# ZKI-PH-ImageAnalysis/seq2squiggle

Measured on AMD Instinct MI355X. Metric: signal samples/sec at 5 kb reads (padded [chunks x 250] samples the predict path emits), higher is better.
Workload: dtype f16x3

## Files before the change

include/s2s_hip.h:

```cpp
#ifndef S2S_HIP_H
#define S2S_HIP_H

#include <stddef.h>
#include <stdint.h>

#ifdef __cplusplus
extern "C" {
#endif

#define S2S_OK 0
#define S2S_ERR_ARG (-1)
#define S2S_ERR_HIP (-2)
#define S2S_ERR_BLOB (-3)
#define S2S_ERR_CODEC (-4)

#define S2S_MODE_F32 0
#define S2S_MODE_F16X3 1
#define S2S_MODE_F16 3
#define S2S_MODE_GENERIC 4
#define S2S_MODE_GENERIC_F16 5
#define S2S_MODE_GENERIC_GEOMETRY 6
#define S2S_MODE_GENERIC_GEOMETRY_F16 7
#define S2S_GEOMETRY_MAX_DNA_LEN 64
#define S2S_GEOMETRY_MAX_SIGNAL_LEN 1024
// ... 252 lines not shown

int64_t s2s_sampler_replay_law(uint32_t* mt_state, const int64_t* contig_ends, int32_t n_contigs,
                               const int64_t* const* n_pos, const int64_t* n_pos_count, int64_t num_seqs, int64_t first_read_i, int64_t r,
                               uint64_t seed, int64_t total_len, int32_t is_dna, int32_t min_read_len, int32_t max_retries,
                               int64_t stop_after, int32_t law, int32_t* out_lengths, int64_t* out_next_read_i);
int64_t s2s_length_law(int32_t law, uint32_t seed, double r, int64_t total_len);

int64_t s2s_fasta_count(const uint8_t* data, int64_t n);
int64_t s2s_fastq_clean(const uint8_t* data, int64_t n, int32_t map_acgtn, uint8_t* out, int64_t* seq_offs,
                        int64_t* name_span, int64_t max_records);
int64_t s2s_fasta_clean(const uint8_t* data, int64_t n, int32_t map_acgtn, uint8_t* out, int64_t* seq_offs,
                        int64_t* name_span, int64_t max_records);

int64_t s2s_copy_ranges(int32_t n, const int32_t* src_fd, const int64_t* src_off, const int32_t* dst_fd, const int64_t* dst_off,
                        const int64_t* len, int32_t threads, int32_t engine);
int64_t s2s_blow5_scan(int32_t fd, int64_t begin, int64_t end);
int64_t s2s_blow5_scan_upto(int32_t fd, int64_t begin, int64_t limit, int64_t max_records, int64_t* out_end);

#define S2S_ATTENTION_REDO_THRESHOLD 0.055
double s2s_attention_redo_threshold(void);
int s2s_set_attention_path(s2s_handle* h, int32_t path);
int s2s_get_attention_path(const s2s_handle* h, int32_t* path, double* calibration_redo_rate);

int s2s_stats_read(s2s_handle* h, uint64_t* out10);

int s2s_diag_read(s2s_handle* h, uint64_t* out384);

#define S2S_TRAINER_DEFAULT_MEMORY ((size_t)2 << 30)
typedef struct s2s_trainer s2s_trainer;
typedef struct s2s_adam {
    double lr, beta1, beta2, eps, weight_decay;
    double clip;
    int32_t decoupled;
    int32_t step;
} s2s_adam;
int s2s_trainer_create(const s2s_config* cfg, const void* weights_blob, size_t blob_bytes, int device, s2s_trainer** out);
void s2s_trainer_destroy(s2s_trainer* t);
const char* s2s_trainer_last_error(const s2s_trainer* t);
int s2s_trainer_set_memory(s2s_trainer* t, size_t bytes);
int64_t s2s_trainer_micro_batch(const s2s_trainer* t, int32_t B);
int s2s_trainer_weights(s2s_trainer* t, void* stream, float* out_blob);
int s2s_trainer_gradients(s2s_trainer* t, void* stream, const uint8_t* kmers, const int32_t* dwell, const float* target,
                          const float* stdev, int32_t B, float* out_loss, float* out_grad);
int s2s_trainer_step(s2s_trainer* t, void* stream, const uint8_t* kmers, const int32_t* dwell, const float* target,
                     const float* stdev, int32_t B, const s2s_adam* hyper, float* out_stats);

// ... 5 lines not shown
```

seq2squiggle_amd/_lib.py:

```python
import ctypes as C
import os

from ._build import LIB as _LIB_DEFAULT

_lib = None
loaded_before_torch = False


class S2SConfig(C.Structure):
    _fields_ = [("seq_kmer", C.c_int32), ("max_dna_len", C.c_int32), ("max_signal_len", C.c_int32),
                ("dmodel", C.c_int32), ("dff", C.c_int32), ("n_heads", C.c_int32), ("encoder_layers", C.c_int32),
                ("decoder_layers", C.c_int32), ("pre_layers", C.c_int32), ("scaling_max_value", C.c_float),
                ("compute_mode", C.c_int32), ("decoder_heads", C.c_int32)]


class S2SParams(C.Structure):
    _fields_ = [("dwell_mean", C.c_float), ("dwell_std", C.c_float), ("noise_std", C.c_float),
                ("min_noise", C.c_float), ("min_duration", C.c_float), ("noise_sampling", C.c_int32),
                ("duration_sampling", C.c_int32), ("seed", C.c_uint64)]


class S2SDebug(C.Structure):
    _fields_ = [(n, C.c_void_p) for n in ("emb_out", "enc_out", "sigma", "conc", "rate", "g", "y_scaled", "z01", "emb_in", "dec_in")]


class S2SAdam(C.Structure):
    _fields_ = [("lr", C.c_double), ("beta1", C.c_double), ("beta2", C.c_double), ("eps", C.c_double), ("weight_decay", C.c_double),
                ("clip", C.c_double), ("decoupled", C.c_int32), ("step", C.c_int32)]


EXPORTS = ("s2s_blob_floats", "s2s_create", "s2s_destroy", "s2s_last_error", "s2s_predict_chunks", "s2s_predict_packed",
           "s2s_export_reads", "s2s_svb_encode", "s2s_philox_u32", "s2s_set_profiling", "s2s_get_kernel_ms", "s2s_stats_read", "s2s_set_attention_path", "s2s_get_attention_path", "s2s_diag_read",
           "s2s_blow5_pack_bound", "s2s_blow5_pack", "s2s_compress_rows", "s2s_sampler_replay", "s2s_sampler_replay_law", "s2s_length_law",
           "s2s_fasta_count", "s2s_fasta_clean", "s2s_fastq_clean", "s2s_copy_ranges", "s2s_blow5_scan", "s2s_blow5_scan_upto", "s2s_attention_redo_threshold", "s2s_evaluate_chunks",
           "s2s_align_chunks", "s2s_paf_format", "s2s_paf_format_bound", "s2s_event_stats", "s2s_events_format", "s2s_events_format_bound",
           "s2s_kmer_table_rows", "s2s_kmer_table_accumulate", "s2s_kmer_table_format", "s2s_kmer_table_format_bound",
           "s2s_event_fixed", "s2s_kmer_model_accumulate", "s2s_kmer_model_format", "s2s_kmer_model_format_bound",
           "s2s_dtw_max_band", "s2s_signal_median_mad", "s2s_signal_normalise", "s2s_dtw_banded",
           "s2s_signal_median_mad_host", "s2s_signal_normalise_host", "s2s_dtw_banded_host",
           "s2s_dtw_path_scratch_bytes", "s2s_dtw_path", "s2s_dtw_path_host",
           "s2s_sdtw_max_query", "s2s_sdtw", "s2s_sdtw_host",
           "s2s_resquiggle_scratch_bytes", "s2s_resquiggle", "s2s_event_sums", "s2s_resquiggle_host", "s2s_event_sums_host",
           "s2s_segment_capacity", "s2s_segment_scratch_bytes", "s2s_segment", "s2s_segment_host", "s2s_segment_format_bound",
           "s2s_segment_format",
           "s2s_eventalign_scratch_bytes", "s2s_event_means", "s2s_eventalign", "s2s_event_means_host", "s2s_eventalign_host",
           "s2s_chunk_scratch_bytes", "s2s_chunk_pack", "s2s_chunk_pack_host",
           "s2s_kmer_model_events", "s2s_kmer_model_events_host",
           "s2s_trainer_create", "s2s_trainer_destroy", "s2s_trainer_last_error", "s2s_trainer_set_memory", "s2s_trainer_micro_batch",
           "s2s_trainer_weights", "s2s_trainer_gradients", "s2s_trainer_step")


def lib():
    global _lib
    if _lib is not None:
        return _lib
# ... 13 lines not shown
            fn = getattr(L, name)
        except AttributeError:
            if lenient:
                return
            raise
        fn.restype, fn.argtypes = restype, argtypes
    bind("s2s_blob_floats", C.c_size_t, [C.POINTER(S2SConfig)])
    bind("s2s_create", i32, [C.POINTER(S2SConfig), vp, C.c_size_t, i32, C.POINTER(vp)])
    bind("s2s_destroy", None, [vp])
    bind("s2s_last_error", C.c_char_p, [vp])
    bind("s2s_predict_chunks", i32, [vp, vp, vp, vp, i64, i32, C.POINTER(S2SParams), vp, vp, vp, vp, vp,
                                     C.POINTER(S2SDebug)])
    bind("s2s_evaluate_chunks", i32, [vp, vp, vp, vp, vp, vp, i32, vp, vp, C.POINTER(S2SDebug)])
    bind("s2s_predict_packed", i32, [vp, vp, vp, vp, vp, i64, i32, C.POINTER(S2SParams), vp, vp])
    bind("s2s_export_reads", i32, [vp, vp, vp, i32, vp, i32, vp, vp, vp, i64, f32, f32, f32, i32])
    bind("s2s_svb_encode", i32, [vp, vp, vp, vp, vp, vp, i32, i64, i32, vp, i64, vp])
    bind("s2s_philox_u32", i32, [vp, vp, u64, u32, u32, u32, u32, i32, vp])
    bind("s2s_set_profiling", i32, [vp, i32])
    bind("s2s_get_kernel_ms", i32, [vp, C.POINTER(C.c_double), C.POINTER(i64), C.POINTER(i64)])
    bind("s2s_stats_read", i32, [vp, C.POINTER(C.c_uint64)])
    bind("s2s_set_attention_path", i32, [vp, i32])
    bind("s2s_get_attention_path", i32, [vp, C.POINTER(i32), C.POINTER(C.c_double)])
    bind("s2s_diag_read", i32, [vp, C.POINTER(C.c_uint64)])
    bind("s2s_blow5_pack_bound", i64, [i64, i32])
    bind("s2s_blow5_pack", i64, [vp, vp, vp, vp, vp, vp, i32, i32, i32, i32, vp, i64])
    bind("s2s_compress_rows", i64, [vp, vp, i32, i32, i32, i32, vp, i64, vp])
    bind("s2s_sampler_replay", i64, [vp, vp, i32, vp, vp, i64, i64, i64, u64, i64, i32, i32, i32, i64, vp, vp])
    bind("s2s_sampler_replay_law", i64, [vp, vp, i32, vp, vp, i64, i64, i64, u64, i64, i32, i32, i32, i64, i32, vp, vp])
    bind("s2s_length_law", i64, [i32, u32, C.c_double, i64])
    bind("s2s_fastq_clean", i64, [vp, i64, i32, vp, vp, vp, i64])
    bind("s2s_fasta_count", i64, [vp, i64])
    bind("s2s_fasta_clean", i64, [vp, i64, i32, vp, vp, vp, i64])
    bind("s2s_copy_ranges", i64, [i32, vp, vp, vp, vp, vp, i32, i32])
    bind("s2s_blow5_scan", i64, [i32, i64, i64])
    bind("s2s_blow5_scan_upto", i64, [i32, i64, i64, i64, C.POINTER(i64)])
    bind("s2s_attention_redo_threshold", C.c_double, [])
    bind("s2s_align_chunks", i32, [vp, vp, vp, vp, i32, vp])
    bind("s2s_paf_format_bound", i64, [i64, i32, i32, i64])
    bind("s2s_paf_format", i64, [vp, i32, vp, vp, vp, i32, vp, vp, i32, i32, i32, vp, i64])
    bind("s2s_event_stats", i32, [vp, vp, vp, vp, i32, f32, f32, f32, vp, vp, vp])
    bind("s2s_events_format_bound", i64, [i64, i32, i64, i32, f32, f32, f32, i64, i32])
    bind("s2s_events_format", i64, [vp, vp, vp, i32, vp, vp, vp, i32, vp, vp, i32, vp, vp, i32, f32, f32, f32, vp, i32, i32, i32, vp, i64])
    bind("s2s_kmer_table_rows", i64, [i32])
    bind("s2s_kmer_table_accumulate", i32, [vp, vp, vp, vp, vp, vp, vp, i32, f32, f32, f32, vp])
    bind("s2s_kmer_table_format_bound", i64, [vp, i32, f32, f32, f32, i32])
    bind("s2s_kmer_table_format", i64, [vp, i32, f32, f32, f32, i32, vp, i64])
# ... 50 lines not shown
```

seq2squiggle_amd/csrc/s2s_device.h:

```cpp
#pragma once
#include <hip/hip_runtime.h>
#include <stdint.h>

typedef float f32x4 __attribute__((ext_vector_type(4)));
typedef float f32x2 __attribute__((ext_vector_type(2)));

#define S2S_MAX_LAYERS 4

struct LayerOff {
    int stream;
    int stream_h;
    int stream_f;
    int bq, bk, bv, bfc, b1, b2;
    int bq_nat, bk_nat;
    int ln1g, ln1b, ln2g, ln2b;
};
struct MlpOff { int w0, b0, w3, b3, w0h; };
struct ModelDev {
    int k, enc_layers, dec_layers, pre_layers;
    float scale;
    int pe_enc, pe_dec;
    int emb_wt, emb_b;
    int pre_w[S2S_MAX_LAYERS], pre_b[S2S_MAX_LAYERS], pre_wh[S2S_MAX_LAYERS];
    LayerOff enc[S2S_MAX_LAYERS], dec[S2S_MAX_LAYERS];
// ... 24 lines not shown
#define DIAG_STAMP(slot)                                                            \
    do {                                                                            \
        __builtin_amdgcn_sched_barrier(0);                                          \
        const unsigned long long n_ = __builtin_readcyclecounter();                 \
        if ((threadIdx.x & 63) == 0) s2s_diag_lds[(threadIdx.x >> 6) * S2S_DIAG_SLOTS + (slot)] += n_ - diag_t_; \
        diag_t_ = n_;                                                               \
        __builtin_amdgcn_sched_barrier(0);                                          \
    } while (0)
#define DIAG_COUNT(slot, n) do { if ((threadIdx.x & 63) == 0) s2s_diag_lds[(threadIdx.x >> 6) * S2S_DIAG_SLOTS + (slot)] += (n); } while (0)
#elif defined(S2S_STAMP_SB)
#define DIAG_DECL
#define DIAG_STAMP(slot) __builtin_amdgcn_sched_barrier(0)
#define DIAG_COUNT(slot, n)
#else
#define DIAG_DECL
#define DIAG_STAMP(slot)
#define DIAG_COUNT(slot, n)
#endif

#define S2S_STAT_REDO 0
#define S2S_STAT_CYCLES 1
#define S2S_STAT_TICKS 2
#define S2S_STAT_WGS 3
__shared__ __attribute__((aligned(256))) unsigned s2s_stats_lds[64];

#ifdef S2S_TILEHIST
__shared__ unsigned s2s_hist_lds[2 * 2 * 64];
#endif
constexpr int S2S_STATIC_LDS_BYTES = 256
#ifdef S2S_DIAG
    + 8 * S2S_DIAG_SLOTS * 8
#endif
#ifdef S2S_TILEHIST
    + 2 * 2 * 64 * 4
#endif
    ;

#ifndef S2S_ABL
#define S2S_ABL 0
#endif
#define MFMA4(a, b, c) __builtin_amdgcn_mfma_f32_16x16x4f32((a), (b), (c), 0, 0, 0)

__device__ __forceinline__ f32x4 ldg4(const float* p) { return *reinterpret_cast<const f32x4*>(p); }
__device__ __forceinline__ void store_stream(float* p, float v) { __hip_atomic_store(p, v, __ATOMIC_RELAXED, __HIP_MEMORY_SCOPE_AGENT); }
__device__ __forceinline__ void store_stream(int* p, int v) { __hip_atomic_store(p, v, __ATOMIC_RELAXED, __HIP_MEMORY_SCOPE_AGENT); }
__device__ __forceinline__ float sum_g(float v) {
    const unsigned u = __float_as_uint(v);
// ... 364 lines not shown
```

seq2squiggle_amd/csrc/s2s_hip.hip:

```cpp
#include "s2s_device.h"
#include "s2s_device_h.h"
#include "s2s_generic.h"
#include "s2s_generic_h.h"
#include "s2s_train.h"
#include "../../include/s2s_hip.h"
#include "s2s_event_fixed.h"
#define S2S_DTW_KERNELS
#include "s2s_dtw.h"
#include "s2s_sdtw.h"
#include "s2s_resquiggle.h"
#include "s2s_prims.h"
#include "s2s_segment.h"
#include "s2s_eventalign.h"
#include "s2s_chunk.h"
#include "s2s_kmer_model_events.h"

#include <cctype>
#include <cstdio>
#include <cstdlib>
#include <cstring>
#include <immintrin.h>
#include <map>
#include <mutex>
#include <string>
// ... 392 lines not shown
                                 ? __fmul_rn(__fmul_rn(fmaxf(se, P.min_noise), P.noise_std), M.scale)
                                 : P.noise_std;
            if (y != 0.0f) y = mul_then_add(z, sd, y);
        }
        store_stream(out_signal + t, fmaxf(y, 0.0f));
    }
}

template <int MODE> struct Fused {
    static constexpr int FMODE = (MODE == 3) ? 1 : MODE;
    static constexpr int FNQ = (FMODE == 1) ? 2 : 1;
    static constexpr int GROUP = DEC_WAVES * FNQ;
    static constexpr bool PF = (MODE == 1);
    static constexpr int LDS = (MODE == 0) ? DEC_LDS_F32 : DEC_LDS_H + (S2S_SLOT_FLOATS + S2S_SV_FLOATS + S2S_PROG_INTS + S2S_Z2_FLOATS) * 4;
    static_assert(LDS + S2S_STATIC_LDS_BYTES + 16 <= 160 * 1024, "LDS per workgroup: dynamic + the static arrays in front of it");
    static_assert(FMODE == 1 || DEC_WAVES * FrontLdsF32::BYTES <= LDS, "the f32 frontend waves' K/V images share the decoder's LDS");
};
#define S2S_MAX_GROUP (2 * DEC_WAVES)
template <int MODE, bool TEST, bool EXACT = false>
__global__ __launch_bounds__(DEC_WAVES * 64, DEC_WPS) void s2s_fused_kernel(
    const ModelDev M, const float* __restrict__ W, const uint8_t* __restrict__ bases,
    const long long* __restrict__ chunk_start, const uint8_t* __restrict__ n_valid, int n_chunks, long long first_chunk,
    ParamsDev P, const float* __restrict__ inj_g_, const float* __restrict__ inj_zdw_, const float* __restrict__ inj_z01_,
    float* __restrict__ handoff, int* __restrict__ out_dur, float* __restrict__ out_signal, DebugDev dbg_, long long dbg_base) {
    using F = Fused<MODE>;
    const float* const inj_g = TEST ? inj_g_ : nullptr;
    const float* const inj_zdw = TEST ? inj_zdw_ : nullptr;
    const float* const inj_z01 = TEST ? inj_z01_ : nullptr;
    DebugDev dbg = dbg_;
    if (!TEST) { dbg = DebugDev{}; dbg.diag = dbg_.diag; dbg.stats = dbg_.stats; }
    extern __shared__ __attribute__((aligned(16))) char lds_raw[];
    const int wave = __builtin_amdgcn_readfirstlane(threadIdx.x >> 6);
    const int lane = threadIdx.x & 63;
    const int nb = S2S_T_ENC + M.k - 1;
    if constexpr (MODE != 0) att32_consts<AttnLdsH<DEC_NQ, DEC_WAVES, DEC_NKT>>(lds_raw, threadIdx.x, DEC_WAVES * 64);
    if constexpr (MODE != 0) {
        if (threadIdx.x < S2S_PROG_INTS + S2S_Z2_FLOATS)
            reinterpret_cast<int*>(lds_raw + DEC_LDS_H + (S2S_SLOT_FLOATS + S2S_SV_FLOATS) * 4)[threadIdx.x] = 0;
    }
    if (threadIdx.x == 0) {
        const unsigned long long c0 = __builtin_readcyclecounter(), r0 = __builtin_amdgcn_s_memrealtime();
        s2s_stats_lds[0] = 0;
        s2s_stats_lds[4] = (unsigned)c0; s2s_stats_lds[5] = (unsigned)(c0 >> 32);
        s2s_stats_lds[6] = (unsigned)r0; s2s_stats_lds[7] = (unsigned)(r0 >> 32);
    }
#ifdef S2S_TILEHIST
    for (int i = threadIdx.x; i < 2 * 2 * 64; i += DEC_WAVES * 64) s2s_hist_lds[i] = 0;
#endif
#ifdef S2S_DIAG
    for (int i = threadIdx.x; i < 8 * S2S_DIAG_SLOTS; i += DEC_WAVES * 64) s2s_diag_lds[i] = 0;
    const unsigned long long diag_c0 = __builtin_readcyclecounter(), diag_r0 = __builtin_amdgcn_s_memrealtime();
    __syncthreads();
#endif
    float* const slot0 = handoff + (size_t)blockIdx.x * S2S_MAX_GROUP * S2S_SLOT_FLOATS;
    const int lo = (int)((long long)blockIdx.x * n_chunks / gridDim.x), hi = (int)((long long)(blockIdx.x + 1) * n_chunks / gridDim.x);
#pragma unroll 1
    for (int g0 = lo; g0 < hi; g0 += F::GROUP) {
        const int n_here = hi - g0 < F::GROUP ? hi - g0 : F::GROUP;
        float one = 1.0f;
        asm volatile("" : "+s"(one));
        DIAG_DECL;
        __syncthreads();
        {
            int lnf = lane;
            asm volatile("" : "+v"(lnf));
            auto chunk_of = [&](const int j, const int j_filler) {
                const bool live = j < n_here;
                const int b = g0 + (live ? j : j_filler);
                return FrontChunk{chunk_start ? bases + chunk_start[b] : bases + (size_t)b * nb, n_valid[b],
                                  (unsigned long long)(first_chunk + b), inj_g ? inj_g + (size_t)b * 16 : nullptr,
                                  inj_zdw ? inj_zdw + (size_t)b * 16 : nullptr, slot0 + j * S2S_SLOT_FLOATS,
                                  out_dur + (size_t)b * 16, dbg_base + b, live};
            };
            if constexpr (F::FMODE == 1) {
                if (n_here > DEC_WAVES) {
                    const FrontChunk io[2] = {chunk_of(2 * wave, 2 * wave), chunk_of(2 * wave + 1, 2 * wave)};
                    if (2 * wave < n_here) frontend_h16<2>(M, W, io, P, dbg, lnf, one);
                } else {
                    const FrontChunk io[1] = {chunk_of(wave, 0)};
                    if (wave < n_here) frontend_h16<1>(M, W, io, P, dbg, lnf, one);
                }
            } else {
                const FrontChunk io[1] = {chunk_of(wave, 0)};
                if (wave < n_here) frontend_f32(M, W, io, P, lds_raw + wave * FrontLdsF32::BYTES, dbg, lnf);
            }
        }
        __syncthreads();
        DIAG_STAMP(7);
        f32x4 X[DEC_NQ][4];
        float sig_ext[DEC_NQ];
        {
            int lg = lane;
            asm volatile("" : "+v"(lg));
            GatherRaw R;
            dec_gather_issue(M, W, slot0, wave, lg, R);
            dec_gather_finish(R, wave, lg, X, sig_ext);
            if (TEST && dbg.dec_in) dec_override(dbg.dec_in, dbg_base + g0, wave, lg, X);
        }
        DIAG_STAMP(8);
#pragma unroll 1
        for (int j = 0; j < ((S2S_ABL & 65536) ? 0 : n_here); ++j) {
            const int b = g0 + j;
            const float* next = slot0 + (j + 1 < n_here ? j + 1 : j) * S2S_SLOT_FLOATS;
            dec_blocks<MODE, EXACT>(M, W, X, lds_raw, wave, lane, one, dbg.diag, F::PF ? next : nullptr);
            DIAG_STAMP(15);
            int ln = lane;
            asm volatile("" : "+v"(ln));
            float ys, se;
            dec_project(M, W, X, sig_ext, ln, ys, se);
            GatherRaw R;
            if constexpr (F::PF) dec_gather_issue(M, W, reinterpret_cast<const float*>(lds_raw + DEC_LDS_H), wave, ln, R);
// ... 5 lines not shown
            DIAG_STAMP(9);
        }
    }
#ifdef S2S_DIAG
    DIAG_COUNT(16, __builtin_readcyclecounter() - diag_c0);
    DIAG_COUNT(17, __builtin_amdgcn_s_memrealtime() - diag_r0);
    DIAG_COUNT(18, 1ull);
    __syncthreads();
    if (dbg.diag)
        for (int i = threadIdx.x; i < 8 * S2S_DIAG_SLOTS; i += DEC_WAVES * 64)
            if (s2s_diag_lds[i]) atomicAdd(dbg.diag + i, s2s_diag_lds[i]);
#endif
    __syncthreads();
#ifdef S2S_TILEHIST
    if (dbg.diag)
        for (int i = threadIdx.x; i < 2 * 2 * 64; i += DEC_WAVES * 64)
            if (s2s_hist_lds[i]) atomicAdd(dbg.diag + i, (unsigned long long)s2s_hist_lds[i]);
#endif
    if (threadIdx.x == 0 && dbg.stats) {
        const unsigned long long c0 = ((unsigned long long)s2s_stats_lds[5] << 32) | s2s_stats_lds[4];
        const unsigned long long r0 = ((unsigned long long)s2s_stats_lds[7] << 32) | s2s_stats_lds[6];
        if (s2s_stats_lds[0]) atomicAdd(dbg.stats + S2S_STAT_REDO, (unsigned long long)s2s_stats_lds[0]);
        atomicAdd(dbg.stats + S2S_STAT_CYCLES, __builtin_readcyclecounter() - c0);
        atomicAdd(dbg.stats + S2S_STAT_TICKS, __builtin_amdgcn_s_memrealtime() - r0);
        atomicAdd(dbg.stats + S2S_STAT_WGS, 1ull);
    }
}

template <int MODE, bool EXACT>
__global__ __launch_bounds__(DEC_WAVES * 64, DEC_WPS) void s2s_eval_kernel(
    const ModelDev M, const float* __restrict__ W, const uint8_t* __restrict__ kmers, const int* __restrict__ dwell, int n_chunks,
    ParamsDev P, float* __restrict__ handoff, float* __restrict__ y, DebugDev dbg_) {
    using F = Fused<MODE>;
    extern __shared__ __attribute__((aligned(16))) char lds_raw[];
    const int wave = __builtin_amdgcn_readfirstlane(threadIdx.x >> 6);
    const int lane = threadIdx.x & 63;
    if constexpr (MODE != 0) att32_consts<AttnLdsH<DEC_NQ, DEC_WAVES, DEC_NKT>>(lds_raw, threadIdx.x, DEC_WAVES * 64);
    if constexpr (MODE != 0) {
        if (threadIdx.x < S2S_PROG_INTS + S2S_Z2_FLOATS)
            reinterpret_cast<int*>(lds_raw + DEC_LDS_H + (S2S_SLOT_FLOATS + S2S_SV_FLOATS) * 4)[threadIdx.x] = 0;
    }
    if (threadIdx.x == 0) s2s_stats_lds[0] = 0;
    DebugDev dbg{};
    dbg.sigma = dbg_.sigma; dbg.conc = dbg_.conc; dbg.rate = dbg_.rate;
    float* const slot0 = handoff + (size_t)blockIdx.x * S2S_MAX_GROUP * S2S_SLOT_FLOATS;
    const int lo = (int)((long long)blockIdx.x * n_chunks / gridDim.x), hi = (int)((long long)(blockIdx.x + 1) * n_chunks / gridDim.x);
    const int kb = S2S_T_ENC * M.k;
#pragma unroll 1
// ... 569 lines not shown

struct s2s_handle {
    s2s_config cfg;
    int device = 0;
    ModelDev model;
    char* slab = nullptr;
    size_t slab_bytes = 0;
    float* d_arena = nullptr;
    size_t arena_floats = 0;
    int tile = 0;
    int n_wg = 256;
    float* handoff = nullptr;
    int* ws_counts = nullptr;
    long long* ws_offs = nullptr;
    int ws_export_cap = 0;
    int* ws_svb = nullptr;
    int ws_svb_cap = 0;
    bool profiling = false;
    unsigned long long* d_diag = nullptr;
    unsigned long long* d_stats = nullptr;
    long long stat_chunks = 0;
    int attn_exact = 0;
    long long stat_exact_chunks = 0;
    double calib_redo_rate = -1.0;
    std::vector<EventPair> events;
    std::string err;
    struct Generic {
        int d = 0, dff = 0, h_enc = 0, h_dec = 0;
        int te = 16, ts = 250;
        bool f16 = false;
        long long pe_enc = 0, pe_dec = 0, emb_wt = 0, emb_b = 0, out_w = 0, out_b = 0, w0cat = 0, b0cat = 0;
        long long pre_w[S2S_MAX_LAYERS] = {}, pre_b[S2S_MAX_LAYERS] = {};
        GenLayer enc[S2S_MAX_LAYERS] = {}, dec[S2S_MAX_LAYERS] = {};
        GenLayerH dech[S2S_MAX_LAYERS] = {};
        GenHeads heads = {};
        int ld_d = 0, ld_f = 0;
        int slice_max = 0;
        float* ws = nullptr;
        int ws_chunks = 0;
    } gen;
    float* ev_ws = nullptr;
    int ev_chunks = 0;
};

namespace {

// ... 515 lines not shown
    if ((e = hipMemcpy(h->d_arena, A.v.data(), h->arena_floats * sizeof(float), hipMemcpyHostToDevice)) != hipSuccess)
        return bail(e, "hipMemcpy(arena)");
    if ((e = hipMemset(h->d_stats, 0, 256)) != hipSuccess) return bail(e, "hipMemset(stats)");
    const struct { const void* fn; int bytes; } dyn_lds[] = {
        {reinterpret_cast<const void*>(s2s_fused_kernel<0, false>), Fused<0>::LDS}, {reinterpret_cast<const void*>(s2s_fused_kernel<1, false>), Fused<1>::LDS},
        {reinterpret_cast<const void*>(s2s_fused_kernel<3, false>), Fused<3>::LDS}, {reinterpret_cast<const void*>(s2s_fused_kernel<0, true>), Fused<0>::LDS},
        {reinterpret_cast<const void*>(s2s_fused_kernel<1, true>), Fused<1>::LDS},  {reinterpret_cast<const void*>(s2s_fused_kernel<3, true>), Fused<3>::LDS},
        {reinterpret_cast<const void*>(s2s_fused_kernel<1, false, true>), Fused<1>::LDS}, {reinterpret_cast<const void*>(s2s_fused_kernel<3, false, true>), Fused<3>::LDS},
        {reinterpret_cast<const void*>(s2s_fused_kernel<1, true, true>), Fused<1>::LDS},  {reinterpret_cast<const void*>(s2s_fused_kernel<3, true, true>), Fused<3>::LDS},
        {reinterpret_cast<const void*>(s2s_eval_kernel<0, false>), Fused<0>::LDS}, {reinterpret_cast<const void*>(s2s_eval_kernel<1, false>), Fused<1>::LDS},
        {reinterpret_cast<const void*>(s2s_eval_kernel<3, false>), Fused<3>::LDS}, {reinterpret_cast<const void*>(s2s_eval_kernel<1, true>), Fused<1>::LDS},
        {reinterpret_cast<const void*>(s2s_eval_kernel<3, true>), Fused<3>::LDS}};
    for (const auto& k : dyn_lds)
        if ((e = hipFuncSetAttribute(k.fn, hipFuncAttributeMaxDynamicSharedMemorySize, k.bytes)) != hipSuccess)
            return bail(e, "hipFuncSetAttribute(dynamic LDS)");
    if (mode_generic(cfg->compute_mode) &&
        (e = hipFuncSetAttribute(reinterpret_cast<const void*>(gen_attention_kernel<true>), hipFuncAttributeMaxDynamicSharedMemorySize,
                                 GEN_ATTN_STAGE_BYTES)) != hipSuccess)
        return bail(e, "hipFuncSetAttribute(generic attention LDS)");
#if defined(S2S_DIAG) || defined(S2S_TILEHIST)
    if ((e = hipMalloc(&h->d_diag, 8 * 48 * sizeof(unsigned long long))) != hipSuccess) return bail(e, "hipMalloc(diag)");
    if ((e = hipMemset(h->d_diag, 0, 8 * 48 * sizeof(unsigned long long))) != hipSuccess) return bail(e, "hipMemset(diag)");
#endif
    std::string want;
    if (const char* env = getenv("S2S_ATTENTION_PATH"))
        for (const char* c = env; *c; ++c) want += (char)std::tolower((unsigned char)*c);
    if (want == "fast" || want == "exact") {
        h->attn_exact = want == "exact" ? 1 : 0;
    } else if (!want.empty() && want != "auto") {
        g_create_error = "S2S_ATTENTION_PATH must be fast, exact or auto (got \"" + want + "\")";
        s2s_destroy(h);
        return S2S_ERR_ARG;
    } else if (calibrate_attention(h) != S2S_OK) {
        g_create_error = "attention-path calibration launch: " + h->err;
        s2s_destroy(h);
        return S2S_ERR_HIP;
    }
    *out = h;
    return S2S_OK;
}

int s2s_set_attention_path(s2s_handle* h, int32_t path) {
    if (!h) return S2S_ERR_ARG;
    if (path != 0 && path != 1) return fail(h, S2S_ERR_ARG, "attention path must be 0 (fast path first) or 1 (exact path)");
    h->attn_exact = path;
    return S2S_OK;
}

int s2s_get_attention_path(const s2s_handle* h, int32_t* path, double* calibration_redo_rate) {
    if (!h) return S2S_ERR_ARG;
    if (path) *path = h->attn_exact;
    if (calibration_redo_rate) *calibration_redo_rate = h->calib_redo_rate;
    return S2S_OK;
}

void s2s_destroy(s2s_handle* h) {
    if (!h) return;
    DeviceGuard guard(h->device);
    for (auto& ev : h->events) { (void)hipEventDestroy(ev.a); (void)hipEventDestroy(ev.b); }
    free_scratch(h, h->ws_counts);
    free_scratch(h, h->ws_offs);
    free_scratch(h, h->ws_svb);
    if (h->gen.ws) (void)hipFree(h->gen.ws);
    if (h->ev_ws) (void)hipFree(h->ev_ws);
    if (h->slab) (void)hipFree(h->slab);
    if (h->d_diag) (void)hipFree(h->d_diag);
    delete h;
}

const char* s2s_last_error(const s2s_handle* h) { return h ? h->err.c_str() : g_create_error.c_str(); }

static int predict_impl(s2s_handle* h, void* stream_, const uint8_t* bases, const int64_t* chunk_start, const uint8_t* n_valid, int64_t first_global_chunk,
                       int32_t B, const s2s_params* params, const float* inject_g, const float* inject_zdw,
                       const float* inject_z01, float* out_signal, int32_t* out_dur, const s2s_debug* dbg) {
    if (!h) return S2S_ERR_ARG;
    if (B < 0) return fail(h, S2S_ERR_ARG, "B < 0");
    if (B == 0) return S2S_OK;
// ... 23 lines not shown
        const int n = (int)((B - s < h->tile) ? (B - s) : h->tile);
        const uint8_t* tb = chunk_start ? bases : bases + (size_t)s * nb;
        const long long* tcs = reinterpret_cast<const long long*>(chunk_start ? chunk_start + s : nullptr);
        const float* tg = inject_g ? inject_g + s * 16 : nullptr;
        const float* tzdw = inject_zdw ? inject_zdw + s * 16 : nullptr;
        const float* tz01 = inject_z01 ? inject_z01 + (size_t)s * S2S_T_DEC : nullptr;
        float* tsig = out_signal + (size_t)s * S2S_T_DEC;
        const long long fc = (long long)(first_global_chunk + s);
        const dim3 grid(n < h->n_wg ? n : h->n_wg), block(DEC_WAVES * 64);
        const int mode = h->cfg.compute_mode;
        EventPair ev{};
        if (h->profiling) {
            HIP_TRY(h, hipEventCreate(&ev.a));
            HIP_TRY(h, hipEventCreate(&ev.b));
            HIP_TRY(h, hipEventRecord(ev.a, stream));
        }
        const bool test = dbg || inject_g || inject_zdw || inject_z01;
        const bool exact = h->attn_exact && mode != S2S_MODE_F32;
        auto fused = exact ? (test ? (mode == S2S_MODE_F16 ? s2s_fused_kernel<3, true, true> : s2s_fused_kernel<1, true, true>)
                                   : (mode == S2S_MODE_F16 ? s2s_fused_kernel<3, false, true> : s2s_fused_kernel<1, false, true>))
                   : test  ? (mode == S2S_MODE_F16 ? s2s_fused_kernel<3, true> : mode == S2S_MODE_F16X3 ? s2s_fused_kernel<1, true> : s2s_fused_kernel<0, true>)
                           : (mode == S2S_MODE_F16 ? s2s_fused_kernel<3, false> : mode == S2S_MODE_F16X3 ? s2s_fused_kernel<1, false> : s2s_fused_kernel<0, false>);
        if (exact) h->stat_exact_chunks += n;
        hipLaunchKernelGGL(fused, grid, block, mode == S2S_MODE_F16 ? Fused<3>::LDS : mode == S2S_MODE_F16X3 ? Fused<1>::LDS : Fused<0>::LDS, stream, h->model, h->d_arena, tb, tcs,
                           n_valid + s, n, fc, P, tg, tzdw, tz01, h->handoff, out_dur + s * 16, tsig, D, (long long)s);
        if (h->profiling) {
            HIP_TRY(h, hipEventRecord(ev.b, stream));
            ev.chunks = n;
            h->events.push_back(ev);
        }
    }
    HIP_TRY(h, hipGetLastError());
    return S2S_OK;
}

#define S2S_EVAL_SLICE 32768

int s2s_evaluate_chunks(s2s_handle* h, void* stream_, const uint8_t* kmers, const int32_t* dwell, const float* target, const float* stdev,
                        int32_t B, float* out_loss, float* out_y, const s2s_debug* dbg) {
    if (!h) return S2S_ERR_ARG;
    if (B < 0) return fail(h, S2S_ERR_ARG, "B < 0");
    if (B == 0) return S2S_OK;
    if (!kmers || !dwell || !target || !stdev || !out_loss) return fail(h, S2S_ERR_ARG, "NULL argument");
    if (dbg && (dbg->emb_in || dbg->dec_in || dbg->emb_out || dbg->enc_out || dbg->g || dbg->y_scaled || dbg->z01))
        return fail(h, S2S_ERR_ARG, "s2s_evaluate_chunks writes only dbg->sigma / conc / rate (and y through out_y)");
    DeviceGuard guard(h->device);
    if (!guard.ok) return fail(h, S2S_ERR_HIP, "hipSetDevice failed");
    hipStream_t st = static_cast<hipStream_t>(stream_);
// ... 254 lines not shown
        (void)hipEventDestroy(ev.a); (void)hipEventDestroy(ev.b);
    }
    h->events.clear();
    if (ms_total) *ms_total = tot;
    if (launches) *launches = nl;
    if (chunks) *chunks = nc;
    return S2S_OK;
}

int s2s_stats_read(s2s_handle* h, uint64_t* out10) {
    if (!h || !out10) return S2S_ERR_ARG;
    DeviceGuard guard(h->device);
    if (!guard.ok) return fail(h, S2S_ERR_HIP, "hipSetDevice failed");
    HIP_TRY(h, hipDeviceSynchronize());
    unsigned long long raw[8];
    HIP_TRY(h, hipMemcpy(raw, h->d_stats, sizeof raw, hipMemcpyDeviceToHost));
    HIP_TRY(h, hipMemset(h->d_stats, 0, sizeof raw));
    out10[0] = (uint64_t)h->stat_chunks;
    out10[1] = mode_generic(h->cfg.compute_mode)
                   ? (uint64_t)h->stat_chunks * (uint64_t)cfg_dec_heads(&h->cfg) * (uint64_t)h->cfg.decoder_layers
                   : (uint64_t)h->stat_chunks * DEC_WAVES * S2S_HEADS * (uint64_t)h->cfg.decoder_layers;
    out10[2] = raw[S2S_STAT_REDO];
    out10[3] = raw[S2S_STAT_CYCLES]; out10[4] = raw[S2S_STAT_TICKS]; out10[5] = raw[S2S_STAT_WGS];
    out10[6] = (uint64_t)h->stat_exact_chunks; out10[7] = 0; out10[8] = 0; out10[9] = 0;
    h->stat_chunks = 0; h->stat_exact_chunks = 0;
    return S2S_OK;
}

int s2s_diag_read(s2s_handle* h, uint64_t* out48) {
    if (!h || !out48) return S2S_ERR_ARG;
    if (!h->d_diag) return fail(h, S2S_ERR_ARG, "not a diagnostic (-DS2S_DIAG) build");
    HIP_TRY(h, hipDeviceSynchronize());
    HIP_TRY(h, hipMemcpy(out48, h->d_diag, 8 * 48 * sizeof(uint64_t), hipMemcpyDeviceToHost));
    HIP_TRY(h, hipMemset(h->d_diag, 0, 8 * 48 * sizeof(uint64_t)));
    return S2S_OK;
}

int32_t s2s_dtw_max_band(void) { return S2S_DTW_MAX_BAND; }

int s2s_signal_median_mad(int device, void* stream_, const int16_t* samples, const int64_t* offs, int32_t R, int32_t* med, int32_t* mad) {
    if (R < 0 || !offs || (R > 0 && (!samples || !med || !mad))) return fail(nullptr, S2S_ERR_ARG, "s2s_signal_median_mad: bad argument");
    if (R == 0) return S2S_OK;
    GUARD_OR_RETURN(nullptr, device);
    S2S_LAUNCH(nullptr, s2s_median_mad_kernel, dim3(R), dim3(S2S_DTW_SELECT_THREADS), 0, static_cast<hipStream_t>(stream_), samples,
               as_ll(offs), med, mad);
    return S2S_OK;
}

// ... 235 lines not shown
```

seq2squiggle_amd/engine.py:

```python
import ctypes as C
import os
from dataclasses import dataclass
from typing import Dict, Optional

import numpy as np
import torch

from . import _lib
from .checkpoint import (DEFAULT_GEOMETRY, GEOMETRY_MODES, TUNED_MODES, TUNED_SIZES, config_to_c, default_mode, is_default_geometry,
                         is_tuned_family, load_checkpoint, state_dict_to_blob)

T_ENC, T_DEC = 16, 250


@dataclass
class PredictParams:
    dwell_mean: float = 12.5
    dwell_std: float = 0.0
    noise_std: float = 2.0
    noise_sampling: bool = True
    duration_sampling: bool = True
    min_noise: float = 0.0
    min_duration: float = 3.0
    seed: int = 0
# ... 384 lines not shown
    def kernel_ms(self):
        ms, nl, nc = C.c_double(), C.c_int64(), C.c_int64()
        self._check(_lib.lib().s2s_get_kernel_ms(self._h, C.byref(ms), C.byref(nl), C.byref(nc)), "s2s_get_kernel_ms")
        return ms.value, nl.value, nc.value

    @property
    def attention_path(self) -> str:
        p, r = C.c_int32(), C.c_double()
        self._check(_lib.lib().s2s_get_attention_path(self._h, C.byref(p), C.byref(r)), "s2s_get_attention_path")
        return "exact" if p.value else "fast"

    @attention_path.setter
    def attention_path(self, path: str):
        if path not in ("fast", "exact"):
            raise ValueError("attention_path must be 'fast' or 'exact'")
        self._check(_lib.lib().s2s_set_attention_path(self._h, int(path == "exact")), "s2s_set_attention_path")

    @property
    def calibration_redo_rate(self) -> float:
        p, r = C.c_int32(), C.c_double()
        self._check(_lib.lib().s2s_get_attention_path(self._h, C.byref(p), C.byref(r)), "s2s_get_attention_path")
        return r.value

    def stats(self) -> dict:
        out = (C.c_uint64 * 10)()
        self._check(_lib.lib().s2s_stats_read(self._h, out), "s2s_stats_read")
        chunks, runs, redo, cyc, ticks, wgs, exact_chunks = (int(x) for x in out[:7])
        return {"chunks": chunks, "softmax_runs": runs, "softmax_redone": redo,
                "redo_rate": (redo / runs) if runs else 0.0,
                "in_kernel_clock_ghz": (cyc / ticks * 0.1) if ticks else None,
                "cycles_per_chunk_and_cu": (cyc / chunks) if chunks else None,
                "shader_cycles": cyc, "ticks_100mhz": ticks, "workgroups": wgs,
                "chunks_on_exact_path": exact_chunks}
```

Baseline: 757.4 million.

## Add dynamic atomic work-claiming schedule with shrinking tail groups to fused kernel

Replaces the fixed per-workgroup contiguous chunk range in the fused predict kernel with an optional dynamic scheduler. Workgroups claim groups of chunks from a global atomic counter, and the claim size shrinks toward single chunks near the tail to balance the load. Auto mode switches to dynamic only when there are at least eight full groups per workgroup. This targets tail imbalance across CUs on large batches, at the cost of an atomic and LDS handoff per group and a counter reset protocol. It also adds per-workgroup span min/max stats.

```diff
diff --git a/include/s2s_hip.h b/include/s2s_hip.h
--- a/include/s2s_hip.h
+++ b/include/s2s_hip.h
@@ -298,6 +298,14 @@
 int s2s_set_attention_path(s2s_handle* h, int32_t path);
 int s2s_get_attention_path(const s2s_handle* h, int32_t* path, double* calibration_redo_rate);
 
+#define S2S_SCHEDULE_AUTO 0
+#define S2S_SCHEDULE_STATIC 1
+#define S2S_SCHEDULE_DYNAMIC 2
+int s2s_set_schedule(s2s_handle* h, int32_t schedule);
+int s2s_get_schedule(const s2s_handle* h, int32_t* schedule);
+void s2s_schedule_claim(int64_t n, int32_t n_wg, int32_t group, int64_t c, int64_t* start, int32_t* count);
+int32_t s2s_schedule_is_dynamic(int64_t n, int32_t n_wg, int32_t group);
+
 int s2s_stats_read(s2s_handle* h, uint64_t* out10);
 
 int s2s_diag_read(s2s_handle* h, uint64_t* out384);
diff --git a/seq2squiggle_amd/_lib.py b/seq2squiggle_amd/_lib.py
--- a/seq2squiggle_amd/_lib.py
+++ b/seq2squiggle_amd/_lib.py
@@ -31,6 +31,7 @@
 
 EXPORTS = ("s2s_blob_floats", "s2s_create", "s2s_destroy", "s2s_last_error", "s2s_predict_chunks", "s2s_predict_packed",
            "s2s_export_reads", "s2s_svb_encode", "s2s_philox_u32", "s2s_set_profiling", "s2s_get_kernel_ms", "s2s_stats_read", "s2s_set_attention_path", "s2s_get_attention_path", "s2s_diag_read",
+           "s2s_set_schedule", "s2s_get_schedule", "s2s_schedule_claim", "s2s_schedule_is_dynamic",
            "s2s_blow5_pack_bound", "s2s_blow5_pack", "s2s_compress_rows", "s2s_sampler_replay", "s2s_sampler_replay_law", "s2s_length_law",
            "s2s_fasta_count", "s2s_fasta_clean", "s2s_fastq_clean", "s2s_copy_ranges", "s2s_blow5_scan", "s2s_blow5_scan_upto", "s2s_attention_redo_threshold", "s2s_evaluate_chunks",
            "s2s_align_chunks", "s2s_paf_format", "s2s_paf_format_bound", "s2s_event_stats", "s2s_events_format", "s2s_events_format_bound",
@@ -90,6 +91,10 @@
     bind("s2s_set_attention_path", i32, [vp, i32])
     bind("s2s_get_attention_path", i32, [vp, C.POINTER(i32), C.POINTER(C.c_double)])
     bind("s2s_diag_read", i32, [vp, C.POINTER(C.c_uint64)])
+    bind("s2s_set_schedule", i32, [vp, i32])
+    bind("s2s_get_schedule", i32, [vp, C.POINTER(i32)])
+    bind("s2s_schedule_claim", None, [i64, i32, i32, i64, C.POINTER(i64), C.POINTER(i32)])
+    bind("s2s_schedule_is_dynamic", i32, [i64, i32, i32])
     bind("s2s_blow5_pack_bound", i64, [i64, i32])
     bind("s2s_blow5_pack", i64, [vp, vp, vp, vp, vp, vp, i32, i32, i32, i32, vp, i64])
     bind("s2s_compress_rows", i64, [vp, vp, i32, i32, i32, i32, vp, i64, vp])
diff --git a/seq2squiggle_amd/csrc/s2s_device.h b/seq2squiggle_amd/csrc/s2s_device.h
--- a/seq2squiggle_amd/csrc/s2s_device.h
+++ b/seq2squiggle_amd/csrc/s2s_device.h
@@ -70,7 +70,15 @@
 #define S2S_STAT_CYCLES 1
 #define S2S_STAT_TICKS 2
 #define S2S_STAT_WGS 3
+#define S2S_STAT_SPAN_MAX 4
+#define S2S_STAT_SPAN_MIN_INV 5
+#define S2S_STAT_SCHED 16
 __shared__ __attribute__((aligned(256))) unsigned s2s_stats_lds[64];
+#define S2S_LDS_G0 8
+#define S2S_LDS_N 9
+#define S2S_LDS_END 10
+#define S2S_LDS_SCHED 11
+#define S2S_LDS_GRID 13
 
 #ifdef S2S_TILEHIST
 __shared__ unsigned s2s_hist_lds[2 * 2 * 64];
diff --git a/seq2squiggle_amd/csrc/s2s_hip.hip b/seq2squiggle_amd/csrc/s2s_hip.hip
--- a/seq2squiggle_amd/csrc/s2s_hip.hip
+++ b/seq2squiggle_amd/csrc/s2s_hip.hip
@@ -1,5 +1,6 @@
 #include "s2s_device.h"
 #include "s2s_device_h.h"
+#include "s2s_schedule.h"
 #include "s2s_generic.h"
 #include "s2s_generic_h.h"
 #include "s2s_train.h"
@@ -438,7 +439,8 @@
     const ModelDev M, const float* __restrict__ W, const uint8_t* __restrict__ bases,
     const long long* __restrict__ chunk_start, const uint8_t* __restrict__ n_valid, int n_chunks, long long first_chunk,
     ParamsDev P, const float* __restrict__ inj_g_, const float* __restrict__ inj_zdw_, const float* __restrict__ inj_z01_,
-    float* __restrict__ handoff, int* __restrict__ out_dur, float* __restrict__ out_signal, DebugDev dbg_, long long dbg_base) {
+    float* __restrict__ handoff, int* __restrict__ out_dur, float* __restrict__ out_signal, DebugDev dbg_, long long dbg_base,
+    unsigned* __restrict__ sched) {
     using F = Fused<MODE>;
     const float* const inj_g = TEST ? inj_g_ : nullptr;
     const float* const inj_zdw = TEST ? inj_zdw_ : nullptr;
@@ -469,14 +471,44 @@
     __syncthreads();
 #endif
     float* const slot0 = handoff + (size_t)blockIdx.x * S2S_MAX_GROUP * S2S_SLOT_FLOATS;
-    const int lo = (int)((long long)blockIdx.x * n_chunks / gridDim.x), hi = (int)((long long)(blockIdx.x + 1) * n_chunks / gridDim.x);
+    auto put_group = [&](const int start, const int count) {
+        s2s_stats_lds[S2S_LDS_G0] = (unsigned)start; s2s_stats_lds[S2S_LDS_N] = (unsigned)count;
+    };
+    auto sched_of = [&]() {
+        return reinterpret_cast<unsigned*>(((unsigned long long)s2s_stats_lds[S2S_LDS_SCHED + 1] << 32) | s2s_stats_lds[S2S_LDS_SCHED]);
+    };
+    auto put_claim = [&](unsigned* const q, const unsigned c) {
+        int start, count;
+        const unsigned G = s2s_stats_lds[S2S_LDS_GRID];
+        s2s_claim_range((int)s2s_stats_lds[S2S_LDS_END], (int)G, F::GROUP, (int)c, &start, &count);
+        put_group(start, count);
+        if (count == 0) {
+            __threadfence();
+            if (atomicInc(q + 1, G - 1) == G - 1) atomicExch(q, 0u);
+        }
+    };
+    if (threadIdx.x == 0) {
+        s2s_stats_lds[S2S_LDS_SCHED] = (unsigned)(unsigned long long)sched;
+        s2s_stats_lds[S2S_LDS_SCHED + 1] = (unsigned)((unsigned long long)sched >> 32);
+        s2s_stats_lds[S2S_LDS_GRID] = gridDim.x;
+        if (sched) {
+            s2s_stats_lds[S2S_LDS_END] = (unsigned)n_chunks;
+            put_claim(sched, atomicAdd(sched, 1u));
+        } else {
+            const int lo = (int)((long long)blockIdx.x * n_chunks / gridDim.x), hi = (int)((long long)(blockIdx.x + 1) * n_chunks / gridDim.x);
+            s2s_stats_lds[S2S_LDS_END] = (unsigned)hi;
+            put_group(lo, hi - lo < F::GROUP ? hi - lo : F::GROUP);
+        }
+    }
 #pragma unroll 1
-    for (int g0 = lo; g0 < hi; g0 += F::GROUP) {
-        const int n_here = hi - g0 < F::GROUP ? hi - g0 : F::GROUP;
+    for (;;) {
         float one = 1.0f;
         asm volatile("" : "+s"(one));
         DIAG_DECL;
         __syncthreads();
+        const int g0 = __builtin_amdgcn_readfirstlane((int)s2s_stats_lds[S2S_LDS_G0]);
+        const int n_here = __builtin_amdgcn_readfirstlane((int)s2s_stats_lds[S2S_LDS_N]);
+        if (n_here <= 0) break;
         {
             int lnf = lane;
             asm volatile("" : "+v"(lnf));
@@ -503,6 +535,14 @@
         }
         __syncthreads();
         DIAG_STAMP(7);
+        if (threadIdx.x == 0) {
+            if (unsigned* const q = sched_of()) {
+                put_claim(q, atomicAdd(q, 1u));
+            } else {
+                const int hi = (int)s2s_stats_lds[S2S_LDS_END], nx = g0 + F::GROUP;
+                put_group(nx, nx >= hi ? 0 : hi - nx < F::GROUP ? hi - nx : F::GROUP);
+            }
+        }
         f32x4 X[DEC_NQ][4];
         float sig_ext[DEC_NQ];
         {
@@ -554,8 +594,11 @@
         const unsigned long long r0 = ((unsigned long long)s2s_stats_lds[7] << 32) | s2s_stats_lds[6];
         if (s2s_stats_lds[0]) atomicAdd(dbg.stats + S2S_STAT_REDO, (unsigned long long)s2s_stats_lds[0]);
         atomicAdd(dbg.stats + S2S_STAT_CYCLES, __builtin_readcyclecounter() - c0);
-        atomicAdd(dbg.stats + S2S_STAT_TICKS, __builtin_amdgcn_s_memrealtime() - r0);
+        const unsigned long long span = __builtin_amdgcn_s_memrealtime() - r0;
+        atomicAdd(dbg.stats + S2S_STAT_TICKS, span);
         atomicAdd(dbg.stats + S2S_STAT_WGS, 1ull);
+        atomicMax(dbg.stats + S2S_STAT_SPAN_MAX, span);
+        atomicMax(dbg.stats + S2S_STAT_SPAN_MIN_INV, ~span);
     }
 }
 
@@ -1171,6 +1214,8 @@
     long long stat_chunks = 0;
     int attn_exact = 0;
     long long stat_exact_chunks = 0;
+    int schedule = S2S_SCHEDULE_AUTO;
+    long long stat_dynamic_chunks = 0;
     double calib_redo_rate = -1.0;
     std::vector<EventPair> events;
     std::string err;
@@ -1732,6 +1777,19 @@
     if ((e = hipMalloc(&h->d_diag, 8 * 48 * sizeof(unsigned long long))) != hipSuccess) return bail(e, "hipMalloc(diag)");
     if ((e = hipMemset(h->d_diag, 0, 8 * 48 * sizeof(unsigned long long))) != hipSuccess) return bail(e, "hipMemset(diag)");
 #endif
+    {
+        std::string sch;
+        if (const char* env = getenv("S2S_SCHEDULE"))
+            for (const char* c = env; *c; ++c) sch += (char)std::tolower((unsigned char)*c);
+        if (sch.empty() || sch == "auto") h->schedule = S2S_SCHEDULE_AUTO;
+        else if (sch == "static") h->schedule = S2S_SCHEDULE_STATIC;
+        else if (sch == "dynamic") h->schedule = S2S_SCHEDULE_DYNAMIC;
+        else {
+            g_create_error = "S2S_SCHEDULE must be auto, static or dynamic (got \"" + sch + "\")";
+            s2s_destroy(h);
+            return S2S_ERR_ARG;
+        }
+    }
     std::string want;
     if (const char* env = getenv("S2S_ATTENTION_PATH"))
         for (const char* c = env; *c; ++c) want += (char)std::tolower((unsigned char)*c);
@@ -1763,6 +1821,30 @@
     if (calibration_redo_rate) *calibration_redo_rate = h->calib_redo_rate;
     return S2S_OK;
 }
+
+int s2s_set_schedule(s2s_handle* h, int32_t schedule) {
+    if (!h) return S2S_ERR_ARG;
+    if (schedule != S2S_SCHEDULE_AUTO && schedule != S2S_SCHEDULE_STATIC && schedule != S2S_SCHEDULE_DYNAMIC)
+        return fail(h, S2S_ERR_ARG, "schedule must be 0 (auto), 1 (static) or 2 (dynamic)");
+    h->schedule = schedule;
+    return S2S_OK;
+}
+
+int s2s_get_schedule(const s2s_handle* h, int32_t* schedule) {
+    if (!h || !schedule) return S2S_ERR_ARG;
+    *schedule = h->schedule;
+    return S2S_OK;
+}
+
+void s2s_schedule_claim(int64_t n, int32_t n_wg, int32_t group, int64_t c, int64_t* start, int32_t* count) {
+    int s = 0, k = 0;
+    if (n >= 0 && n <= (1 << 30) && n_wg > 0 && group > 0 && (int64_t)n_wg * group <= (1 << 30) && c >= 0 && c < (1ll << 31))
+        s2s_claim_range((int)n, n_wg, group, (int)c, &s, &k);
+    if (start) *start = s;
+    if (count) *count = k;
+}
+
+int32_t s2s_schedule_is_dynamic(int64_t n, int32_t n_wg, int32_t group) { return s2s_auto_takes_claims(n, n_wg, group) ? 1 : 0; }
 
 void s2s_destroy(s2s_handle* h) {
     if (!h) return;
@@ -1832,8 +1914,12 @@
                    : test  ? (mode == S2S_MODE_F16 ? s2s_fused_kernel<3, true> : mode == S2S_MODE_F16X3 ? s2s_fused_kernel<1, true> : s2s_fused_kernel<0, true>)
                            : (mode == S2S_MODE_F16 ? s2s_fused_kernel<3, false> : mode == S2S_MODE_F16X3 ? s2s_fused_kernel<1, false> : s2s_fused_kernel<0, false>);
         if (exact) h->stat_exact_chunks += n;
+        const bool dynamic = h->schedule == S2S_SCHEDULE_DYNAMIC ||
+                             (h->schedule == S2S_SCHEDULE_AUTO && s2s_auto_takes_claims(n, h->n_wg, mode == S2S_MODE_F32 ? Fused<0>::GROUP : Fused<1>::GROUP));
+        if (dynamic) h->stat_dynamic_chunks += n;
+        unsigned* const sched = dynamic ? reinterpret_cast<unsigned*>(h->d_stats + S2S_STAT_SCHED) : nullptr;
         hipLaunchKernelGGL(fused, grid, block, mode == S2S_MODE_F16 ? Fused<3>::LDS : mode == S2S_MODE_F16X3 ? Fused<1>::LDS : Fused<0>::LDS, stream, h->model, h->d_arena, tb, tcs,
-                           n_valid + s, n, fc, P, tg, tzdw, tz01, h->handoff, out_dur + s * 16, tsig, D, (long long)s);
+                           n_valid + s, n, fc, P, tg, tzdw, tz01, h->handoff, out_dur + s * 16, tsig, D, (long long)s, sched);
         if (h->profiling) {
             HIP_TRY(h, hipEventRecord(ev.b, stream));
             ev.chunks = n;
@@ -2134,8 +2220,11 @@
                    : (uint64_t)h->stat_chunks * DEC_WAVES * S2S_HEADS * (uint64_t)h->cfg.decoder_layers;
     out10[2] = raw[S2S_STAT_REDO];
     out10[3] = raw[S2S_STAT_CYCLES]; out10[4] = raw[S2S_STAT_TICKS]; out10[5] = raw[S2S_STAT_WGS];
-    out10[6] = (uint64_t)h->stat_exact_chunks; out10[7] = 0; out10[8] = 0; out10[9] = 0;
-    h->stat_chunks = 0; h->stat_exact_chunks = 0;
+    out10[6] = (uint64_t)h->stat_exact_chunks;
+    out10[7] = raw[S2S_STAT_SPAN_MAX];
+    out10[8] = raw[S2S_STAT_SPAN_MIN_INV] ? ~raw[S2S_STAT_SPAN_MIN_INV] : 0;
+    out10[9] = (uint64_t)h->stat_dynamic_chunks;
+    h->stat_chunks = 0; h->stat_exact_chunks = 0; h->stat_dynamic_chunks = 0;
     return S2S_OK;
 }
 
diff --git a/seq2squiggle_amd/csrc/s2s_schedule.h b/seq2squiggle_amd/csrc/s2s_schedule.h
--- /dev/null
+++ b/seq2squiggle_amd/csrc/s2s_schedule.h
@@ -0,0 +1,32 @@
+#pragma once
+
+#if defined(__HIPCC__) || defined(__CUDACC__)
+#define S2S_HD __host__ __device__
+#else
+#define S2S_HD
+#endif
+
+#define S2S_SCHEDULE_AUTO_GROUPS 8
+
+S2S_HD inline void s2s_claim_range(const int n, const int G, const int group, const int c, int* start, int* count) {
+    if (c < 0 || n <= 0) { *start = n > 0 ? n : 0; *count = 0; return; }
+    const int full = G * group;
+    const int H = n > full ? (n - full) / group : 0;
+    if (c < H) { *start = c * group; *count = group; return; }
+    const int Z = n - H * group;
+    int idx = c - H, pos = H * group;
+    for (int s = group >> 1; s >= 2; s >>= 1) {
+        const int above = Z - G * s;
+        int cs = above > 0 ? above / s : 0;
+        if (cs > G) cs = G;
+        if (idx < cs) { *start = pos + idx * s; *count = s; return; }
+        idx -= cs;
+        pos += cs * s;
+    }
+    if (idx < n - pos) { *start = pos + idx; *count = 1; return; }
+    *start = n; *count = 0;
+}
+
+S2S_HD inline bool s2s_auto_takes_claims(const long long n, const int G, const int group) {
+    return n >= (long long)S2S_SCHEDULE_AUTO_GROUPS * G * group;
+}
diff --git a/seq2squiggle_amd/engine.py b/seq2squiggle_amd/engine.py
--- a/seq2squiggle_amd/engine.py
+++ b/seq2squiggle_amd/engine.py
@@ -430,13 +430,30 @@
         self._check(_lib.lib().s2s_get_attention_path(self._h, C.byref(p), C.byref(r)), "s2s_get_attention_path")
         return r.value
 
+    _SCHEDULES = ("auto", "static", "dynamic")
+
+    @property
+    def schedule(self) -> str:
+        v = C.c_int32()
+        self._check(_lib.lib().s2s_get_schedule(self._h, C.byref(v)), "s2s_get_schedule")
+        return self._SCHEDULES[v.value]
+
+    @schedule.setter
+    def schedule(self, schedule: str):
+        if schedule not in self._SCHEDULES:
+            raise ValueError("schedule must be 'auto', 'static' or 'dynamic'")
+        self._check(_lib.lib().s2s_set_schedule(self._h, self._SCHEDULES.index(schedule)), "s2s_set_schedule")
+
     def stats(self) -> dict:
         out = (C.c_uint64 * 10)()
         self._check(_lib.lib().s2s_stats_read(self._h, out), "s2s_stats_read")
-        chunks, runs, redo, cyc, ticks, wgs, exact_chunks = (int(x) for x in out[:7])
+        chunks, runs, redo, cyc, ticks, wgs, exact_chunks, span_max, span_min, dynamic_chunks = (int(x) for x in out[:10])
         return {"chunks": chunks, "softmax_runs": runs, "softmax_redone": redo,
                 "redo_rate": (redo / runs) if runs else 0.0,
                 "in_kernel_clock_ghz": (cyc / ticks * 0.1) if ticks else None,
                 "cycles_per_chunk_and_cu": (cyc / chunks) if chunks else None,
                 "shader_cycles": cyc, "ticks_100mhz": ticks, "workgroups": wgs,
-                "chunks_on_exact_path": exact_chunks}
+                "chunks_on_exact_path": exact_chunks,
+                "wg_span_ms_mean": (ticks / wgs * 1e-5) if wgs else 0.0,
+                "wg_span_ms_max": span_max * 1e-5, "wg_span_ms_min": span_min * 1e-5,
+                "chunks_on_dynamic_schedule": dynamic_chunks}
```

Measured after the change: 766.1 million, median of 6. 1.01x the previous value.
